# qdrant/quantization

Hardware: AMD Instinct MI355X
Metric: scored vectors/sec, 10Mx768 u8 dot (higher is better)
Workload: dtype u8; 1 GPU; 10000000 x 768 store: f32 U[0,1) -> scalar u8 (dot); per step: encode_query + score_all over the shard; quantizer=u8, rows_per_gpu=10000000, dim=768, distance=dot, exchange=scores, gather_group=1, launch=single rank, world_size_seen=1, encode_ahead=False, total_rows=10000000, queries=16

## Files before the change

### quantization_amd/csrc/u8.hip

```cpp
#include <algorithm>
#include <cmath>
#include <cstdlib>
#include <memory>
#include <vector>

#include "common.hpp"
#include "lists.hpp"
#include "multi_reduce.hpp"
#include "topk.hpp"
#include "topk_device.hpp"
#include "rescore.hpp"
#include "u8_internal.hpp"

#pragma clang fp contract(off)

using namespace qamd;

namespace {

constexpr int kBlock = 256;
constexpr int kScanBlock = 512;
constexpr uint64_t kRowPad = 1024;
constexpr uint64_t kQuantileSample = 100000;

enum Epilogue : int { EPI_POINT = 0, EPI_INTERNAL = 1 };

typedef uint32_t u32x4 __attribute__((ext_vector_type(4)));
typedef float f32x4 __attribute__((ext_vector_type(4)));

__device__ __forceinline__ uint4 ld_nt(const uint4 *p) {
    u32x4 t = __builtin_nontemporal_load(reinterpret_cast<const u32x4 *>(p));
    return make_uint4(t.x, t.y, t.z, t.w);
}
__device__ __forceinline__ float4 ld_nt(const float4 *p) {
    f32x4 t = __builtin_nontemporal_load(reinterpret_cast<const f32x4 *>(p));
    return make_float4(t.x, t.y, t.z, t.w);
}

__device__ __forceinline__ uint32_t dot16(const uint4 &a, const uint4 &b, uint32_t acc) {
    acc = __builtin_amdgcn_udot4(a.x, b.x, acc, false);
    acc = __builtin_amdgcn_udot4(a.y, b.y, acc, false);
    acc = __builtin_amdgcn_udot4(a.z, b.z, acc, false);
    acc = __builtin_amdgcn_udot4(a.w, b.w, acc, false);
    return acc;
}

__device__ __forceinline__ uint32_t sad16(const uint4 &a, const uint4 &b, uint32_t acc) {
    acc = __builtin_amdgcn_sad_u8(a.x, b.x, acc);
    acc = __builtin_amdgcn_sad_u8(a.y, b.y, acc);
    acc = __builtin_amdgcn_sad_u8(a.z, b.z, acc);
    acc = __builtin_amdgcn_sad_u8(a.w, b.w, acc);
    return acc;
}

template <int CTRL> __device__ __forceinline__ uint32_t dpp_add(uint32_t v) {
    return v + (uint32_t)__builtin_amdgcn_update_dpp(0, (int)v, CTRL, 0xF, 0xF, false);
}
template <int G> __device__ __forceinline__ uint32_t group_sum(uint32_t v) {
    static_assert(G == 1 || G == 2 || G == 4 || G == 8 || G == 16, "row group is at most one DPP row");
    if (G >= 2) v = dpp_add<0xB1>(v);
    if (G >= 4) v = dpp_add<0x4E>(v);
    if (G >= 8) v = dpp_add<0x141>(v);
    if (G >= 16) v = dpp_add<0x140>(v);
    return v;
}

__device__ __forceinline__ float epilogue_f(float multiplier, float sf, float q_off, float v_off, float diff, int mode) {
    float ms = multiplier * sf;
    if (mode == EPI_POINT) return (ms + q_off) + v_off;
    return ms + ((q_off + v_off) - diff);
}
__device__ __forceinline__ float epilogue(float multiplier, uint32_t s, float q_off, float v_off,
                                          float diff, int mode) {
    return epilogue_f(multiplier, (float)(int32_t)s, q_off, v_off, diff, mode);
}

__device__ __forceinline__ void dot16_lanes(const uint4 &v, const uint4 &q, uint32_t (&acc)[8]) {
    const uint32_t vd[4] = {v.x, v.y, v.z, v.w};
    const uint32_t qd[4] = {q.x, q.y, q.z, q.w};
#pragma unroll
    for (int j = 0; j < 4; j++) {
        acc[2 * j] = __builtin_amdgcn_udot4(vd[j], qd[j] & 0x0000FFFFu, acc[2 * j], false);
        acc[2 * j + 1] = __builtin_amdgcn_udot4(vd[j], qd[j] & 0xFFFF0000u, acc[2 * j + 1], false);
    }
}
template <int G> __device__ __forceinline__ float avx2_lane_sum(uint32_t (&acc)[8]) {
    float f[8];
#pragma unroll
    for (int k = 0; k < 8; k++) f[k] = (float)(int32_t)group_sum<G>(acc[k]);
    float a0 = f[0] + f[4], a1 = f[1] + f[5], a2 = f[2] + f[6], a3 = f[3] + f[7];
    return (a0 + a2) + (a1 + a3);
}

__device__ __forceinline__ uint32_t f32_to_u8(float v, float alpha, float offset) {
    float x = (v - offset) / alpha;
    x = (x < 0.0f) ? 0.0f : x;
    x = (x > 127.0f) ? 127.0f : x;
    return (x != x) ? 0u : (uint32_t)x;
}

__device__ __forceinline__ bool quant_decided(float y) {
    constexpr float kBand = 3.0517578125e-05f;
    const float fr = __builtin_amdgcn_fractf(y);
    return (__builtin_fabsf(fr - 0.5f) <= 0.5f - kBand) || (__builtin_fabsf(y - 64.0f) >= 64.0f + kBand);
}
__device__ __forceinline__ uint32_t quant_code(float y) {
    return (uint32_t)__builtin_amdgcn_fmed3f(y, 0.0f, 127.0f);
}
__device__ __forceinline__ uint32_t f32x4_to_u8x4_fast(const float4 &f, float alpha, float offset, float r_alpha) {
    const float y0 = (f.x - offset) * r_alpha, y1 = (f.y - offset) * r_alpha, y2 = (f.z - offset) * r_alpha,
                y3 = (f.w - offset) * r_alpha;
    if (quant_decided(y0) && quant_decided(y1) && quant_decided(y2) && quant_decided(y3))
        return quant_code(y0) | (quant_code(y1) << 8) | (quant_code(y2) << 16) | (quant_code(y3) << 24);
    return f32_to_u8(f.x, alpha, offset) | (f32_to_u8(f.y, alpha, offset) << 8) | (f32_to_u8(f.z, alpha, offset) << 16) |
           (f32_to_u8(f.w, alpha, offset) << 24);
}

template <int G, int ITERS, int UNROLL, bool IS_L1, bool EXACT, bool FILTER, bool PACKED = false>
__global__ __launch_bounds__(kScanBlock) void u8_scan_kernel(
    const uint4 *__restrict__ codes, const float *__restrict__ offsets,
    const uint4 *__restrict__ qcodes, const float *__restrict__ q_off_p, float multiplier,
    uint32_t n_rows, uint32_t row_chunks, uint32_t n_extra, float *__restrict__ out, TopkFilter filt) {
    static_assert(!(PACKED && IS_L1), "the packed image serves Dot and L2 only");
    constexpr int RW = 64 / G;
    constexpr int TILE = RW * UNROLL;
    const int lane = threadIdx.x & 63;
    const int sub = lane % G;
    const int rslot = lane / G;
    const uint64_t wave = ((uint64_t)blockIdx.x * kScanBlock + threadIdx.x) >> 6;
    const uint64_t base = wave * TILE;
    if (base >= n_rows) return;

    uint4 v[UNROLL][ITERS];
#pragma unroll
    for (int u = 0; u < UNROLL; u++) {
        const uint64_t row = base + u * RW + rslot;
        const uint4 *p = codes + row * row_chunks;
#pragma unroll
        for (int it = 0; it < ITERS; it++) {
            const uint32_t c = sub + it * G;
            if (EXACT) {
                v[u][it] = ld_nt(p + c);
            } else if (PACKED) {
                v[u][it] = ld_nt(p + (it < ITERS - 1 || c < row_chunks ? c : row_chunks - 1));
            } else {
                const uint32_t cc = c < row_chunks ? c : row_chunks - 1;
                uint4 t = ld_nt(p + cc);
                const bool in = c < row_chunks;
                v[u][it] = make_uint4(in ? t.x : 0, in ? t.y : 0, in ? t.z : 0, in ? t.w : 0);
            }
        }
    }
    uint4 q[ITERS];
#pragma unroll
    for (int it = 0; it < ITERS; it++) {
        const uint32_t c = sub + it * G;
        if (EXACT) {
            q[it] = qcodes[c];
        } else {
            const uint4 t = qcodes[c < row_chunks ? c : row_chunks - 1];
            const bool in = c < row_chunks;
            q[it] = make_uint4(in ? t.x : 0, in ? t.y : 0, in ? t.z : 0, in ? t.w : 0);
        }
    }
    uint4 qx[PACKED ? ITERS : 1];
    uint32_t qsh[PACKED ? ITERS : 1];
    if (PACKED) {
#pragma unroll
        for (int it = 0; it < ITERS; it++) {
            const uint32_t c = sub + it * G, e = c / 7;
            const bool has = c < 7 * n_extra;
            const uint4 t = qcodes[has ? row_chunks + e : 0];
            qx[it] = make_uint4(has ? t.x : 0, has ? t.y : 0, has ? t.z : 0, has ? t.w : 0);
            qsh[it] = 7 - (c - 7 * e);
        }
    }
    const float q_off = *q_off_p;
    constexpr int NGROUPS = (UNROLL + G - 1) / G;
    float v_off[NGROUPS];
#pragma unroll
    for (int g = 0; g < NGROUPS; g++)
        v_off[g] = offsets[base + (uint64_t)(g * G + sub) * RW + rslot];
    float mine = 0.0f;
    uint32_t pivot = 0;
    if (FILTER) pivot = *filt.pivot_key;
#pragma unroll
    for (int u = 0; u < UNROLL; u++) {
        uint32_t acc = 0;
#pragma unroll
        for (int it = 0; it < ITERS; it++) {
            if (PACKED) {
                const uint4 &w = v[u][it];
                const uint32_t hi = dot16(make_uint4(w.x & 0x80808080u, w.y & 0x80808080u, w.z & 0x80808080u,
                                                     w.w & 0x80808080u), qx[it], 0);
                acc = dot16(make_uint4(w.x & 0x7F7F7F7Fu, w.y & 0x7F7F7F7Fu, w.z & 0x7F7F7F7Fu, w.w & 0x7F7F7F7Fu),
                            q[it], acc) + (hi >> qsh[it]);
            } else {
                acc = IS_L1 ? sad16(v[u][it], q[it], acc) : dot16(v[u][it], q[it], acc);
            }
        }
        acc = group_sum<G>(acc);
        if (sub == (u % G)) mine = epilogue(multiplier, acc, q_off, v_off[u / G], 0.0f, EPI_POINT);
        if ((u % G) == G - 1 || u == UNROLL - 1) {
            constexpr int dummy = 0;
            (void)dummy;
            const int first = (u / G) * G;
            const uint64_t row = base + (uint64_t)(first + sub) * RW + rslot;
            if (sub <= u - first && row < n_rows) {
                if (FILTER) topk_offer(filt, pivot, mine, (uint32_t)row);
                else __builtin_nontemporal_store(mine, out + row);
            }
        }
    }
}

template <int G, int ITERS, int UNROLL, int NQ, bool IS_L1, bool EXACT, bool FILTER>
__global__ __launch_bounds__(kScanBlock) void u8_scan_multi_kernel(
    const uint4 *__restrict__ codes, const float *__restrict__ offsets, const uint8_t *__restrict__ qcodes,
    uint32_t q_pitch, const float *__restrict__ q_offs, uint32_t nq_valid ,
    float multiplier, uint32_t n_rows, uint32_t row_chunks, float *__restrict__ out ,
    uint64_t out_pitch, TopkFilterSlices slices) {
    static_assert(G >= NQ, "one lane of the row group per query");
    constexpr int RW = 64 / G;
    constexpr int TILE = RW * UNROLL;
    constexpr int TPW = NQ;
    const int lane = threadIdx.x & 63;
    const int sub = lane % G, rslot = lane / G;
    const uint64_t wave = ((uint64_t)blockIdx.x * kScanBlock + threadIdx.x) >> 6;
    if (wave * TILE * TPW >= n_rows) return;
    uint4 q[NQ][ITERS];
#pragma unroll
    for (int j = 0; j < NQ; j++) {
        const uint4 *qj = reinterpret_cast<const uint4 *>(qcodes + (size_t)((uint32_t)j < nq_valid ? j : nq_valid - 1) * q_pitch);
#pragma unroll
        for (int it = 0; it < ITERS; it++) {
            const uint32_t c = sub + it * G;
            const bool in = EXACT || c < row_chunks;
            const uint4 t = qj[in ? c : row_chunks - 1];
            q[j][it] = make_uint4(in ? t.x : 0, in ? t.y : 0, in ? t.z : 0, in ? t.w : 0);
        }
    }
    const int my_q = multi_query_of<NQ>(sub);
    const bool owner = sub < NQ && (uint32_t)my_q < nq_valid;
    const float q_off = q_offs[owner ? my_q : 0];
    for (int tile = 0; tile < TPW; tile++) {
        const uint64_t base = (wave * TPW + tile) * TILE;
        if (base >= n_rows) break;
        uint4 v[UNROLL][ITERS];
#pragma unroll
        for (int u = 0; u < UNROLL; u++) {
            const uint4 *p = codes + (base + u * RW + rslot) * row_chunks;
#pragma unroll
            for (int it = 0; it < ITERS; it++) {
                const uint32_t c = sub + it * G;
                const bool in = EXACT || c < row_chunks;
                const uint4 t = ld_nt(p + (in ? c : row_chunks - 1));
                v[u][it] = make_uint4(in ? t.x : 0, in ? t.y : 0, in ? t.z : 0, in ? t.w : 0);
            }
        }
#pragma unroll
        for (int u = 0; u < UNROLL; u++) {
            const uint64_t row = base + (uint64_t)u * RW + rslot;
            const float v_off = offsets[row];
            uint32_t acc[NQ];
#pragma unroll
            for (int j = 0; j < NQ; j++) {
                acc[j] = 0;
#pragma unroll
                for (int it = 0; it < ITERS; it++)
                    acc[j] = IS_L1 ? sad16(v[u][it], q[j][it], acc[j]) : dot16(v[u][it], q[j][it], acc[j]);
            }
            const float mine = epilogue(multiplier, multi_reduce<G, NQ>(acc, sub), q_off, v_off, 0.0f, EPI_POINT);
            if (owner && row < n_rows) {
                if (FILTER) {
                    const TopkFilter f = topk_filter_of(slices, (uint32_t)my_q);
                    topk_offer(f, *f.pivot_key, mine, (uint32_t)row);
                } else {
                    __builtin_nontemporal_store(mine, out + (uint64_t)my_q * out_pitch + row);
                }
            }
        }
    }
}

template <int G, int ITERS, bool IS_L1, bool EXACT>
__device__ __forceinline__ void u8_topk_small_body(const uint4 *__restrict__ codes, const float *__restrict__ offsets,
                                                   const uint4 (&q)[ITERS], float q_off, float multiplier, uint32_t n_rows,
                                                   uint32_t row_chunks, uint32_t rows_per_wg, const SmallTopk &p,
                                                   unsigned long long (*lds)[64]) {
    unsigned long long(*lists)[64] = lds;
    constexpr int RW = 64 / G;
    constexpr int UNROLL = 2;
    const int lane = threadIdx.x & 63, wave = threadIdx.x >> 6;
    const int sub = lane % G, rslot = lane / G;
    unsigned long long *stage = lds[kSmallTopkWaves + wave];
// ... 558 lines not shown
#pragma unroll
    for (int m = 1; m < 64; m <<= 1) {
        s1 += __shfl_xor(s1, m, 64);
        s2 += __shfl_xor(s2, m, 64);
    }
    if (lane == 0) {
        float off;
        if (distance == QAMD_DOT) {
            float s = (float)s1;
            if (s1 >= (1u << 24)) {
                s = 0.0f;
                for (uint32_t j = 0; j < actual_dim; j++)
                    s += (float)(j < qdim ? f32_to_u8(query[j], alpha, offset) : pad_code);
            }
            off = s * alpha * offset;
        } else if (distance == QAMD_L1) {
            off = 0.0f;
        } else {
            float s = (float)s2;
            if (s2 >= (1u << 24)) {
                s = 0.0f;
                for (uint32_t j = 0; j < actual_dim; j++) {
                    float c = (float)(j < qdim ? f32_to_u8(query[j], alpha, offset) : pad_code);
                    s += c * c;
                }
            }
            off = s * alpha * alpha;
        }
        offsets_out[blockIdx.x] = invert ? -off : off;
    }
}

__global__ __launch_bounds__(kBlock) void split_rows_kernel(const uint32_t *__restrict__ rows32,
                                                           uint64_t n_rows, uint32_t row_dwords,
                                                           uint32_t *__restrict__ codes32,
                                                           float *__restrict__ offsets) {
    const uint64_t total = n_rows * row_dwords;
    const uint64_t stride = (uint64_t)gridDim.x * kBlock;
    for (uint64_t t = (uint64_t)blockIdx.x * kBlock + threadIdx.x; t < total; t += stride) {
        uint64_t r = t / row_dwords;
        uint32_t k = (uint32_t)(t - r * row_dwords);
        uint32_t w = rows32[t];
        if (k == 0)
            offsets[r] = __uint_as_float(w);
        else
            codes32[r * (row_dwords - 1) + (k - 1)] = w;
    }
}

__global__ __launch_bounds__(kBlock) void join_rows_kernel(const uint32_t *__restrict__ codes32,
                                                          const float *__restrict__ offsets,
                                                          uint64_t n_rows, uint32_t row_dwords,
                                                          uint32_t *__restrict__ rows32) {
    const uint64_t total = n_rows * row_dwords;
    const uint64_t stride = (uint64_t)gridDim.x * kBlock;
    for (uint64_t t = (uint64_t)blockIdx.x * kBlock + threadIdx.x; t < total; t += stride) {
        uint64_t r = t / row_dwords;
        uint32_t k = (uint32_t)(t - r * row_dwords);
        rows32[t] = k == 0 ? __float_as_uint(offsets[r]) : codes32[r * (row_dwords - 1) + (k - 1)];
    }
}

__global__ __launch_bounds__(kBlock) void u8_pack7_kernel(const uint4 *__restrict__ codes, uint64_t n_rows,
                                                          uint32_t row_chunks, uint32_t pchunks, uint32_t n_extra,
                                                          uint4 *__restrict__ packed, uint32_t *__restrict__ bad) {
    const uint64_t total = n_rows * pchunks, stride = (uint64_t)gridDim.x * kBlock;
    uint32_t high = 0;
    for (uint64_t t = (uint64_t)blockIdx.x * kBlock + threadIdx.x; t < total; t += stride) {
        const uint64_t r = t / pchunks;
        const uint32_t j = (uint32_t)(t - r * pchunks);
        const uint4 *row = codes + r * row_chunks;
        const uint4 a = row[j];
        uint32_t w[4] = {a.x & 0x7F7F7F7Fu, a.y & 0x7F7F7F7Fu, a.z & 0x7F7F7F7Fu, a.w & 0x7F7F7F7Fu};
        high |= a.x | a.y | a.z | a.w;
        if (j < 7 * n_extra) {
            const uint4 x = row[pchunks + j / 7];
            const uint32_t b = j % 7;
            high |= x.x | x.y | x.z | x.w;
            w[0] |= ((x.x >> b) & 0x01010101u) << 7;
            w[1] |= ((x.y >> b) & 0x01010101u) << 7;
            w[2] |= ((x.z >> b) & 0x01010101u) << 7;
            w[3] |= ((x.w >> b) & 0x01010101u) << 7;
        }
        packed[t] = make_uint4(w[0], w[1], w[2], w[3]);
    }
    if (high & 0x80808080u) atomicOr(bad, 1u);
}

int grid_for(uint64_t work_items, uint64_t per_block, int blocks_per_cu) {
    uint64_t want = (work_items + per_block - 1) / per_block;
    uint64_t cap = (uint64_t)device_info().cu_count * blocks_per_cu;
    if (want < 1) want = 1;
    return (int)(want > cap ? cap : want);
}

float host_multiplier(float alpha, int distance, int invert) {
    float m = distance == QAMD_DOT ? alpha * alpha : distance == QAMD_L1 ? alpha : -2.0f * alpha * alpha;
    return invert ? -m : m;
}

uint64_t actual_dim_of(uint64_t dim) { return dim + (16 - dim % 16) % 16; }

}


namespace {

qamd_status alloc_store(qamd_u8 *h) {
    h->padded_rows = round_up(h->count, kRowPad) + kRowPad;
    h->row_chunks = (uint32_t)(h->meta.actual_dim / 16);
    QAMD_TRY(h->codes.alloc_zero_tail(h->padded_rows * h->meta.actual_dim, h->count * h->meta.actual_dim));
    QAMD_TRY(h->offsets.alloc_zero_tail(h->padded_rows * sizeof(float), h->count * sizeof(float)));
    return QAMD_OK;
}

qamd_status build_packed(qamd_u8 *h, hipStream_t s) {
    h->packed.release();
    h->packed_chunks = 0;
    const uint32_t rc = h->row_chunks, n_extra = rc / 8, pchunks = rc - n_extra;
    if (!u8_packed_allowed() || h->count == 0 || rc < 8 || rc > 128 ||
        h->meta.vector_parameters.distance_type == QAMD_L1)
        return QAMD_OK;
    const uint64_t bytes = h->padded_rows * pchunks * 16;
    size_t free_b = 0, total_b = 0;
    if (hipMemGetInfo(&free_b, &total_b) != hipSuccess || free_b < 2 * bytes) {
        (void)hipGetLastError();
        return QAMD_OK;
    }
    DevBuf img, bad;
    const std::string err = last_error();
    if (img.alloc_zero_tail(bytes, h->count * pchunks * 16) != QAMD_OK || bad.alloc(sizeof(uint32_t), true) != QAMD_OK) {
        (void)hipGetLastError();
        last_error() = err;
        return QAMD_OK;
    }
    hipLaunchKernelGGL(u8_pack7_kernel, dim3(grid_for(h->count * pchunks, kBlock, 8)), dim3(kBlock), 0, s,
                       h->codes.as<uint4>(), h->count, rc, pchunks, n_extra, img.as<uint4>(), bad.as<uint32_t>());
    QAMD_HIP(hipGetLastError());
    uint32_t high = 0;
    QAMD_HIP(hipMemcpyAsync(&high, bad.ptr, sizeof(high), hipMemcpyDeviceToHost, s));
    QAMD_HIP(hipStreamSynchronize(s));
    if (high) return QAMD_OK;
    h->packed = std::move(img);
    h->packed_chunks = pchunks;
    return QAMD_OK;
}

template <bool IS_L1> struct ScanLaunch {
    template <int G, int ITERS, int UNROLL>
    static void go(const qamd_u8 *h, bool packed, uint32_t chunks, const uint4 *qc, const float *qo, float *out,
                   const TopkFilter *filt, hipStream_t s) {
        constexpr int TILE = (64 / G) * UNROLL;
        const uint64_t waves = (h->count + TILE - 1) / TILE;
        const unsigned grid = (unsigned)((waves + kScanBlock / 64 - 1) / (kScanBlock / 64));
        const bool exact = chunks == (uint32_t)(G * ITERS);
        const uint4 *codes = packed ? h->packed.as<uint4>() : h->codes.as<uint4>();
        const uint32_t n_extra = h->row_chunks - chunks;
#define QAMD_U8_GO(EX, FI, PK)                                                                                  \
    hipLaunchKernelGGL((u8_scan_kernel<G, ITERS, UNROLL, IS_L1, EX, FI, PK>), dim3(grid),                      \
                       dim3(kScanBlock), 0, s, codes, h->offsets.as<float>(), qc, qo, h->meta.multiplier,          \
                       (uint32_t)h->count, chunks, n_extra, out, filt ? *filt : TopkFilter{})
        if constexpr (!IS_L1) {
            if (packed) {
                if (filt) {
                    if (exact) QAMD_U8_GO(true, true, true);
                    else QAMD_U8_GO(false, true, true);
                } else {
                    if (exact) QAMD_U8_GO(true, false, true);
                    else QAMD_U8_GO(false, false, true);
                }
                return;
            }
        }
        if (filt) {
            if (exact) QAMD_U8_GO(true, true, false);
            else QAMD_U8_GO(false, true, false);
        } else {
            if (exact) QAMD_U8_GO(true, false, false);
            else QAMD_U8_GO(false, false, false);
        }
#undef QAMD_U8_GO
    }
};

template <bool IS_L1>
bool launch_scan(const qamd_u8 *h, const uint4 *qc, const float *qo, float *out, const TopkFilter *filt,
                 hipStream_t s) {
    using L = ScanLaunch<IS_L1>;
    const bool packed = !IS_L1 && h->packed_chunks != 0;
    const uint32_t rc = packed ? h->packed_chunks : h->row_chunks;
    h->last_scan_packed.store(packed ? 1 : 0, std::memory_order_relaxed);
    if (rc == 1) return L::template go<1, 1, 4>(h, packed, rc, qc, qo, out, filt, s), true;
    if (rc == 2) return L::template go<2, 1, 4>(h, packed, rc, qc, qo, out, filt, s), true;
    if (rc <= 4) return L::template go<4, 1, 8>(h, packed, rc, qc, qo, out, filt, s), true;
    if (rc <= 8) return L::template go<8, 1, 8>(h, packed, rc, qc, qo, out, filt, s), true;
    switch ((rc + 15) / 16) {
        case 1: return L::template go<16, 1, 8>(h, packed, rc, qc, qo, out, filt, s), true;
        case 2: return L::template go<16, 2, 4>(h, packed, rc, qc, qo, out, filt, s), true;
        case 3: return L::template go<16, 3, 4>(h, packed, rc, qc, qo, out, filt, s), true;
        case 4: return L::template go<16, 4, 2>(h, packed, rc, qc, qo, out, filt, s), true;
        case 5: return L::template go<16, 5, 2>(h, packed, rc, qc, qo, out, filt, s), true;
        case 6: return L::template go<16, 6, 2>(h, packed, rc, qc, qo, out, filt, s), true;
        case 7: return L::template go<16, 7, 2>(h, packed, rc, qc, qo, out, filt, s), true;
        case 8: return L::template go<16, 8, 2>(h, packed, rc, qc, qo, out, filt, s), true;
        default: break;
    }
    return false;
}

template <bool IS_L1>
void launch_scan_generic(const qamd_u8 *h, const uint4 *qc, const float *qo, float *out, hipStream_t s) {
    uint64_t waves = (h->count + 3) / 4;
    unsigned grid = (unsigned)((waves + kBlock / 64 - 1) / (kBlock / 64));
    hipLaunchKernelGGL((u8_scan_generic_kernel<IS_L1>), dim3(grid), dim3(kBlock), 0, s,
                       h->codes.as<uint4>(), h->offsets.as<float>(), qc, qo, h->meta.multiplier,
                       (uint32_t)h->count, h->row_chunks, out);
}

template <bool IS_L1> struct SmallLaunch {
    template <int G, int ITERS>
    static qamd_status go(const qamd_u8 *h, const uint4 *qc, const float *qo, const FusedQuery *fq, const SmallTopkPlan &pl,
                          const SmallTopk &p, hipStream_t s) {
        const bool exact = h->row_chunks == (uint32_t)(G * ITERS);
        if constexpr (G * ITERS * 16 > (int)kFusedQueryDims + 15 * 16) {
            if (fq) return fail(QAMD_ERR_ARGUMENTS, "fused query does not fit the kernel arguments");
        } else if (fq) {
            QueryByValue qv;
            memcpy(qv.v, fq->values, (size_t)fq->qdim * 4);
            const qamd_vector_parameters &vp = h->meta.vector_parameters;
#define QAMD_U8_SMALL_FUSED(EX)                                                                                        \
    hipLaunchKernelGGL((u8_topk_small_fused_kernel<G, ITERS, IS_L1, EX>), dim3(pl.workgroups), dim3(1024), 0, s,          \
                       h->codes.as<uint4>(), h->offsets.as<float>(), qv, fq->qdim, (uint32_t)h->meta.actual_dim,         \
                       h->meta.alpha, h->meta.offset, vp.distance_type, vp.invert, fq->qbuf, h->meta.multiplier,           \
                       (uint32_t)h->count, h->row_chunks, pl.rows_per_wg, p)
            if (exact) QAMD_U8_SMALL_FUSED(true);
            else QAMD_U8_SMALL_FUSED(false);
#undef QAMD_U8_SMALL_FUSED
            QAMD_HIP(hipGetLastError());
            return QAMD_OK;
        }
#define QAMD_U8_SMALL(EX)                                                                                       \
    hipLaunchKernelGGL((u8_topk_small_kernel<G, ITERS, IS_L1, EX>), dim3(pl.workgroups), dim3(1024), 0, s,       \
                       h->codes.as<uint4>(), h->offsets.as<float>(), qc, qo, h->meta.multiplier, (uint32_t)h->count, \
                       h->row_chunks, pl.rows_per_wg, p)
        if (exact) QAMD_U8_SMALL(true);
        else QAMD_U8_SMALL(false);
#undef QAMD_U8_SMALL
        QAMD_HIP(hipGetLastError());
        return QAMD_OK;
    }
};

int small_group(uint32_t rc) { return rc == 1 ? 1 : rc == 2 ? 2 : rc <= 4 ? 4 : rc <= 8 ? 8 : rc <= 128 ? 16 : 0; }

template <bool IS_L1>
qamd_status launch_small(const qamd_u8 *h, const uint4 *qc, const float *qo, const FusedQuery *fq, const SmallTopkPlan &pl,
                         const SmallTopk &p, hipStream_t s) {
    using L = SmallLaunch<IS_L1>;
    const uint32_t rc = h->row_chunks;
    h->last_scan_packed.store(0, std::memory_order_relaxed);
    if (rc == 1) return L::template go<1, 1>(h, qc, qo, fq, pl, p, s);
    if (rc == 2) return L::template go<2, 1>(h, qc, qo, fq, pl, p, s);
    if (rc <= 4) return L::template go<4, 1>(h, qc, qo, fq, pl, p, s);
    if (rc <= 8) return L::template go<8, 1>(h, qc, qo, fq, pl, p, s);
    switch ((rc + 15) / 16) {
        case 1: return L::template go<16, 1>(h, qc, qo, fq, pl, p, s);
        case 2: return L::template go<16, 2>(h, qc, qo, fq, pl, p, s);
        case 3: return L::template go<16, 3>(h, qc, qo, fq, pl, p, s);
        case 4: return L::template go<16, 4>(h, qc, qo, fq, pl, p, s);
        case 5: return L::template go<16, 5>(h, qc, qo, fq, pl, p, s);
        case 6: return L::template go<16, 6>(h, qc, qo, fq, pl, p, s);
        case 7: return L::template go<16, 7>(h, qc, qo, fq, pl, p, s);
        case 8: return L::template go<16, 8>(h, qc, qo, fq, pl, p, s);
        default: break;
    }
    return fail(QAMD_ERR_ARGUMENTS, "no small top-k kernel for %u chunks", rc);
}

template <bool IS_L1, int G, int ITERS, int UNROLL, int NQ>
void launch_multi_shape(const qamd_u8 *h, const uint8_t *qcodes, uint64_t q_pitch, const float *q_offs, uint32_t nq_valid,
                        float *out, const TopkFilterSlices *slices, hipStream_t s) {
    constexpr int TILE = (64 / G) * UNROLL * NQ;
    const uint64_t waves = (h->count + TILE - 1) / TILE;
    const unsigned grid = (unsigned)((waves + kScanBlock / 64 - 1) / (kScanBlock / 64));
    const bool exact = h->row_chunks == (uint32_t)(G * ITERS);
    h->last_scan_packed.store(0, std::memory_order_relaxed);
#define QAMD_U8_MULTI(EX, FI)                                                                                      \
// ... 1028 lines not shown
                                uint32_t n_queries, uint32_t k, int largest, uint32_t *out_ids, float *out_scores,
                                qamd_mem out_mem, hipStream_t stream) {
    auto qc = [&](uint32_t q) { return reinterpret_cast<const uint4 *>(codes_dev + (uint64_t)q * pitch); };
    BatchScan scan;
    scan.filter_capable = fused_capable(h);
    scan.scan_scores = [&](uint32_t q, float *scores, hipStream_t st) { return scan_ptrs(h, qc(q), offsets_dev + q, scores, st); };
    scan.scan_filter = [&](uint32_t q, const TopkFilter &f, hipStream_t st) {
        return scan_ptrs(h, qc(q), offsets_dev + q, nullptr, st, &f);
    };
    scan.score_ids = [&](uint32_t q, const uint32_t *ids, uint64_t n_ids, float *out, hipStream_t st) {
        return score_ids_dev(h, qc(q), offsets_dev + q, 0.0f, EPI_POINT, ids, n_ids, out, st);
    };
    const bool is_l1 = h->meta.vector_parameters.distance_type == QAMD_L1;
    const uint32_t width = multi_width(h);
    if (width)
        scan.scan_filter_multi = [&, width, is_l1](uint32_t q, uint32_t left, const TopkFilterSlices &sl, hipStream_t st,
                                                   qamd_status &status) -> uint32_t {
            const uint32_t nq = std::min(left, width);
            if (nq < 2) return 0;
            const uint8_t *qcodes = codes_dev + (uint64_t)q * pitch;
            const bool ok = is_l1 ? launch_multi<true>(h, nq, qcodes, pitch, offsets_dev + q, nullptr, &sl, st)
                                  : launch_multi<false>(h, nq, qcodes, pitch, offsets_dev + q, nullptr, &sl, st);
            if (ok && hipGetLastError() != hipSuccess) status = fail(QAMD_ERR_DEVICE, "u8 multi-query filter launch failed");
            return ok ? nq : 0;
        };
    return fused_topk_batch(h->count, n_queries, k, largest, out_ids, out_scores, out_mem, stream, scan);
}

bool u8_host_encode_is_lazy(uint64_t qdim) { return qdim > 0 && actual_dim_of(qdim) <= kFusedQueryDims; }

qamd_status u8_score_lists(const qamd_u8 *h, const uint8_t *codes_dev, uint64_t pitch, const float *offsets_dev,
                           const ListArgs &a, hipStream_t stream) {
    return score_pairs_dev(h, nullptr, nullptr, codes_dev, (uint32_t)pitch, offsets_dev, a.offsets, a.n_lists, nullptr, 0.0f,
                           EPI_POINT, a.ids, a.n_pairs, a.out, stream);
}

uint32_t u8_multi_width(const qamd_u8 *h) { return multi_width(h); }

bool u8_lane_order(const qamd_u8 *h) { return lane_order(h); }

qamd_status u8_score_batch_scans(const qamd_u8 *h, const uint8_t *codes_dev, uint64_t pitch, const float *offsets_dev,
                                 uint32_t n_queries, float *out_dev, hipStream_t stream) {
    const bool is_l1 = h->meta.vector_parameters.distance_type == QAMD_L1;
    const uint32_t width = multi_width(h);
    uint32_t q = 0;
    while (q < n_queries) {
        const uint32_t nq = std::min(width, n_queries - q);
        const uint8_t *qcodes = codes_dev + (uint64_t)q * pitch;
        float *o = out_dev + (uint64_t)q * h->count;
        const bool ok = nq >= 2 && (is_l1 ? launch_multi<true>(h, nq, qcodes, pitch, offsets_dev + q, o, nullptr, stream)
                                          : launch_multi<false>(h, nq, qcodes, pitch, offsets_dev + q, o, nullptr, stream));
        if (ok) {
            q += nq;
        } else {
            QAMD_TRY(scan_ptrs(h, reinterpret_cast<const uint4 *>(qcodes), offsets_dev + q, o, stream));
            q += 1;
        }
    }
    QAMD_HIP(hipGetLastError());
    return QAMD_OK;
}

qamd_status u8_topk_single(const qamd_u8 *h, const uint8_t *codes_dev, const float *offset_dev, uint32_t k,
                           int largest, uint32_t *out_ids, float *out_scores, qamd_mem out_mem, hipStream_t stream) {
    return u8_topk_ptrs(h, codes_dev, offset_dev, k, largest, out_ids, out_scores, out_mem, stream, nullptr);
}

qamd_status u8_score_single(const qamd_u8 *h, const uint8_t *codes_dev, const float *offset_dev, float *out_dev,
                            hipStream_t stream) {
    return scan_ptrs(h, reinterpret_cast<const uint4 *>(codes_dev), offset_dev, out_dev, stream);
}

}

#ifdef QAMD_DEV
extern "C" __attribute__((visibility("default"))) void qamd_dev_u8_ptrs(const qamd_u8 *h, const void **codes,
                                                                        const void **offsets) {
    *codes = h->codes.ptr;
    *offsets = h->offsets.ptr;
}
extern "C" __attribute__((visibility("default"))) const void *qamd_dev_u8_query_ptr(const qamd_u8_query *q) {
    return q->buf.ptr;
}
extern "C" __attribute__((visibility("default"))) void qamd_dev_u8_packed(const qamd_u8 *h, const void **packed,
                                                                          uint32_t *chunks) {
    *packed = h->packed.ptr;
    *chunks = h->packed_chunks;
}
extern "C" __attribute__((visibility("default"))) int qamd_dev_u8_last_scan_packed(const qamd_u8 *h) {
    return h->last_scan_packed.load(std::memory_order_relaxed);
}
#endif

extern "C" qamd_status qamd_u8_topk_rescored(const qamd_u8 *h, const qamd_u8_query *q, const qamd_f32 *orig,
                                              const float *query_f32, uint64_t qdim, qamd_mem query_mem, uint32_t k,
                                              uint32_t candidates, int largest, uint32_t *out_ids, float *out_scores,
                                              qamd_mem out_mem, void *stream) {
    if (!h || !q) return qamd::fail(QAMD_ERR_ARGUMENTS, "null handle or query");
    return qamd::topk_rescored(h->device, h->meta.vector_parameters, orig, query_f32, 1, qdim, query_mem, k, candidates, largest, out_ids,
                               out_scores, out_mem, qamd::as_stream(stream), [&](uint32_t *ids_dev, float *scores_dev) {
                                   return qamd_u8_topk(h, q, candidates, largest, ids_dev, scores_dev, QAMD_MEM_DEVICE, stream);
                               });
}
```

### quantization_amd/csrc/u8_internal.hpp

```cpp
#pragma once
#include <atomic>
#include <mutex>

#include "common.hpp"
#include "lists.hpp"

struct qamd_u8 {
    int device = 0;
    qamd_u8_metadata meta{};
    uint64_t count = 0;
    uint64_t padded_rows = 0;
    uint32_t row_chunks = 0;
    int lane_mode = 0;
    qamd::DevBuf codes;
    qamd::DevBuf offsets;
    qamd::DevBuf packed;
    uint32_t packed_chunks = 0;
    mutable std::atomic<int> last_scan_packed{0};
    mutable std::mutex sample_mu;
    mutable qamd::DevBuf sample_codes, sample_offsets;
    mutable uint32_t sample_rows = 0;
};

struct qamd_u8_query {
    int device = 0;
    uint64_t actual_dim = 0;
    qamd::DevBuf buf;
    mutable qamd::ReadyEvent ready;
    mutable std::vector<float> host_f32;
    float alpha = 0.0f, offset = 0.0f;
    int distance = 0, invert = 0;
    mutable std::atomic<bool> deferred{false};
    mutable std::mutex encode_mu;
    bool pooled = false;
    mutable std::atomic<bool> async_used{false};
    ~qamd_u8_query() {
        if (pooled) qamd::query_buf_put(buf, !async_used.load(std::memory_order_relaxed) && ready.complete());
    }
};

namespace qamd {
qamd_status u8_minmax_range(const float *data, qamd_mem mem, uint64_t n_rows, uint64_t dim, hipStream_t s, float *mn,
                            float *mx);
qamd_status u8_quantile_interval(const float *data, qamd_mem mem, uint64_t count, uint64_t dim, float quantile,
                                 hipStream_t s, bool *found, float *mn, float *mx);
}

namespace qamd {
qamd_status u8_encode_queries_device(const qamd_u8 *h, const float *queries_dev, uint64_t n_queries, uint64_t qdim,
                                     uint8_t *codes_dev , uint64_t code_pitch,
                                     float *offsets_dev ,
                                     hipStream_t stream);
bool u8_host_encode_is_lazy(uint64_t qdim);
struct FusedQuery {
    const float *values = nullptr;
    uint32_t qdim = 0;
    uint8_t *qbuf = nullptr;
};
qamd_status u8_topk_ptrs(const qamd_u8 *h, const uint8_t *codes_dev, const float *offset_dev, uint32_t k, int largest,
                         uint32_t *out_ids, float *out_scores, qamd_mem out_mem, hipStream_t stream,
                         const FusedQuery *fq = nullptr);
qamd_status u8_topk_batch_scans(const qamd_u8 *h, const uint8_t *codes_dev, uint64_t pitch, const float *offsets_dev,
                                uint32_t n_queries, uint32_t k, int largest, uint32_t *out_ids, float *out_scores,
                                qamd_mem out_mem, hipStream_t stream);
uint32_t u8_multi_width(const qamd_u8 *h);
bool u8_lane_order(const qamd_u8 *h);
qamd_status u8_score_batch_scans(const qamd_u8 *h, const uint8_t *codes_dev, uint64_t pitch, const float *offsets_dev,
                                 uint32_t n_queries, float *out_dev, hipStream_t stream);
qamd_status u8_score_single(const qamd_u8 *h, const uint8_t *codes_dev, const float *offset_dev, float *out_dev,
                            hipStream_t stream);
qamd_status u8_score_lists(const qamd_u8 *h, const uint8_t *codes_dev, uint64_t pitch, const float *offsets_dev,
                           const ListArgs &a, hipStream_t stream);
qamd_status u8_topk_single(const qamd_u8 *h, const uint8_t *codes_dev, const float *offset_dev, uint32_t k,
                           int largest, uint32_t *out_ids, float *out_scores, qamd_mem out_mem, hipStream_t stream);
}
```

Baseline: 9.635 billion vectors/s.

## Store packed u8 image in 64-row blocked layout and scan with dedicated kernel

```diff
diff --git a/quantization_amd/csrc/u8.hip b/quantization_amd/csrc/u8.hip
--- a/quantization_amd/csrc/u8.hip
+++ b/quantization_amd/csrc/u8.hip
@@ -2,6 +2,7 @@
 #include <cmath>
 #include <cstdlib>
 #include <memory>
+#include <type_traits>
 #include <vector>
 
 #include "common.hpp"
@@ -116,12 +117,11 @@
            (f32_to_u8(f.w, alpha, offset) << 24);
 }
 
-template <int G, int ITERS, int UNROLL, bool IS_L1, bool EXACT, bool FILTER, bool PACKED = false>
+template <int G, int ITERS, int UNROLL, bool IS_L1, bool EXACT, bool FILTER>
 __global__ __launch_bounds__(kScanBlock) void u8_scan_kernel(
     const uint4 *__restrict__ codes, const float *__restrict__ offsets,
     const uint4 *__restrict__ qcodes, const float *__restrict__ q_off_p, float multiplier,
-    uint32_t n_rows, uint32_t row_chunks, uint32_t n_extra, float *__restrict__ out, TopkFilter filt) {
-    static_assert(!(PACKED && IS_L1), "the packed image serves Dot and L2 only");
+    uint32_t n_rows, uint32_t row_chunks, float *__restrict__ out, TopkFilter filt) {
     constexpr int RW = 64 / G;
     constexpr int TILE = RW * UNROLL;
     const int lane = threadIdx.x & 63;
@@ -141,8 +141,6 @@
             const uint32_t c = sub + it * G;
             if (EXACT) {
                 v[u][it] = ld_nt(p + c);
-            } else if (PACKED) {
-                v[u][it] = ld_nt(p + (it < ITERS - 1 || c < row_chunks ? c : row_chunks - 1));
             } else {
                 const uint32_t cc = c < row_chunks ? c : row_chunks - 1;
                 uint4 t = ld_nt(p + cc);
@@ -163,18 +161,6 @@
             q[it] = make_uint4(in ? t.x : 0, in ? t.y : 0, in ? t.z : 0, in ? t.w : 0);
         }
     }
-    uint4 qx[PACKED ? ITERS : 1];
-    uint32_t qsh[PACKED ? ITERS : 1];
-    if (PACKED) {
-#pragma unroll
-        for (int it = 0; it < ITERS; it++) {
-            const uint32_t c = sub + it * G, e = c / 7;
-            const bool has = c < 7 * n_extra;
-            const uint4 t = qcodes[has ? row_chunks + e : 0];
-            qx[it] = make_uint4(has ? t.x : 0, has ? t.y : 0, has ? t.z : 0, has ? t.w : 0);
-            qsh[it] = 7 - (c - 7 * e);
-        }
-    }
     const float q_off = *q_off_p;
     constexpr int NGROUPS = (UNROLL + G - 1) / G;
     float v_off[NGROUPS];
@@ -188,17 +174,7 @@
     for (int u = 0; u < UNROLL; u++) {
         uint32_t acc = 0;
 #pragma unroll
-        for (int it = 0; it < ITERS; it++) {
-            if (PACKED) {
-                const uint4 &w = v[u][it];
-                const uint32_t hi = dot16(make_uint4(w.x & 0x80808080u, w.y & 0x80808080u, w.z & 0x80808080u,
-                                                     w.w & 0x80808080u), qx[it], 0);
-                acc = dot16(make_uint4(w.x & 0x7F7F7F7Fu, w.y & 0x7F7F7F7Fu, w.z & 0x7F7F7F7Fu, w.w & 0x7F7F7F7Fu),
-                            q[it], acc) + (hi >> qsh[it]);
-            } else {
-                acc = IS_L1 ? sad16(v[u][it], q[it], acc) : dot16(v[u][it], q[it], acc);
-            }
-        }
+        for (int it = 0; it < ITERS; it++) acc = IS_L1 ? sad16(v[u][it], q[it], acc) : dot16(v[u][it], q[it], acc);
         acc = group_sum<G>(acc);
         if (sub == (u % G)) mine = epilogue(multiplier, acc, q_off, v_off[u / G], 0.0f, EPI_POINT);
         if ((u % G) == G - 1 || u == UNROLL - 1) {
@@ -211,6 +187,83 @@
                 else __builtin_nontemporal_store(mine, out + row);
             }
         }
+    }
+}
+
+constexpr uint32_t kPackBlockRows = 64;
+constexpr uint32_t kPackBlockChunk = kPackBlockRows;
+
+__device__ __forceinline__ uint4 and16(const uint4 &v, uint32_t m) { return make_uint4(v.x & m, v.y & m, v.z & m, v.w & m); }
+
+template <bool FILTER>
+__global__ __launch_bounds__(kScanBlock) __attribute__((amdgpu_waves_per_eu(8, 8))) void u8_scan_blocked_kernel(
+    const uint4 *__restrict__ image, const float *__restrict__ offsets, const uint4 *__restrict__ qcodes,
+    const float *__restrict__ q_off_p, float multiplier, uint32_t n_rows, uint32_t pchunks, uint32_t n_extra,
+    uint32_t split, float *__restrict__ out, TopkFilter filt) {
+    __shared__ uint32_t partial[kScanBlock];
+    const uint32_t lane = threadIdx.x & 63;
+    const uint32_t wave = __builtin_amdgcn_readfirstlane(threadIdx.x >> 6);
+    const uint32_t part = wave & (split - 1);
+    const uint64_t block = (uint64_t)blockIdx.x * ((kScanBlock / 64) / split) + wave / split;
+    const uint64_t row = block * kPackBlockRows + lane;
+    const bool live = block * kPackBlockRows < n_rows;
+    const uint32_t n_rest = pchunks - 7 * n_extra, n_groups = n_extra + (n_rest ? 1 : 0);
+    const uint32_t g_begin = live ? n_groups * part / split : 0, g_end = live ? n_groups * (part + 1) / split : 0;
+    const uint4 *blk = image + block * pchunks * kPackBlockChunk;
+    const uint32_t lane16 = lane * 16;
+    auto chunk_ptr = [&](uint32_t c) {
+        return reinterpret_cast<const uint4 *>(reinterpret_cast<const char *>(blk + (uint64_t)c * kPackBlockChunk) + lane16);
+    };
+    const uint32_t gf_end = g_end < n_extra ? g_end : n_extra;
+    const bool has_rest = g_end > n_extra;
+
+    uint4 v[7];
+    uint32_t acc = 0;
+    auto eat = [&](uint32_t g, auto refill) {
+        const uint4 *q = qcodes + 7 * g;
+        const uint4 qx = qcodes[pchunks + g];
+#pragma unroll
+        for (int i = 0; i < 7; i++) {
+            const uint4 w = v[i];
+            acc = dot16(and16(w, 0x7F7F7F7Fu), q[i], acc) + (dot16(and16(w, 0x80808080u), qx, 0) >> (7 - i));
+            if (decltype(refill)::value) {
+                __builtin_amdgcn_sched_barrier(0);
+                v[i] = ld_nt(chunk_ptr(7 * (g + 1) + i));
+                __builtin_amdgcn_sched_barrier(0);
+            }
+        }
+    };
+    if (g_begin < gf_end) {
+#pragma unroll
+        for (int i = 0; i < 7; i++) v[i] = ld_nt(chunk_ptr(7 * g_begin + i));
+    }
+    const float v_off = offsets[row];
+    const float q_off = *q_off_p;
+    uint32_t pivot = 0;
+    if (FILTER) pivot = *filt.pivot_key;
+    if (g_begin < gf_end) {
+        for (uint32_t g = g_begin; g + 1 < gf_end; g++) eat(g, std::true_type{});
+        eat(gf_end - 1, std::false_type{});
+    }
+    if (has_rest) {
+        const uint4 *q = qcodes + 7 * n_extra;
+#pragma unroll
+        for (int i = 0; i < 7; i++)
+            if ((uint32_t)i < n_rest) v[i] = ld_nt(chunk_ptr(7 * n_extra + i));
+#pragma unroll
+        for (int i = 0; i < 7; i++)
+            if ((uint32_t)i < n_rest) acc = dot16(and16(v[i], 0x7F7F7F7Fu), q[i], acc);
+    }
+    if (split > 1) {
+        partial[threadIdx.x] = acc;
+        __syncthreads();
+        if (part == 0)
+            for (uint32_t p = 1; p < split; p++) acc += partial[threadIdx.x + 64 * p];
+    }
+    if (part == 0 && row < n_rows) {
+        const float score = epilogue(multiplier, acc, q_off, v_off, 0.0f, EPI_POINT);
+        if (FILTER) topk_offer(filt, pivot, score, (uint32_t)row);
+        else __builtin_nontemporal_store(score, out + row);
     }
 }
 
@@ -935,7 +988,7 @@
             w[2] |= ((x.z >> b) & 0x01010101u) << 7;
             w[3] |= ((x.w >> b) & 0x01010101u) << 7;
         }
-        packed[t] = make_uint4(w[0], w[1], w[2], w[3]);
+        packed[((r / kPackBlockRows) * pchunks + j) * kPackBlockRows + r % kPackBlockRows] = make_uint4(w[0], w[1], w[2], w[3]);
     }
     if (high & 0x80808080u) atomicOr(bad, 1u);
 }
@@ -969,6 +1022,7 @@
 
 qamd_status build_packed(qamd_u8 *h, hipStream_t s) {
     h->packed.release();
+    h->packed_rows.release();
     h->packed_chunks = 0;
     const uint32_t rc = h->row_chunks, n_extra = rc / 8, pchunks = rc - n_extra;
     if (!u8_packed_allowed() || h->count == 0 || rc < 8 || rc > 128 ||
@@ -982,7 +1036,7 @@
     }
     DevBuf img, bad;
     const std::string err = last_error();
-    if (img.alloc_zero_tail(bytes, h->count * pchunks * 16) != QAMD_OK || bad.alloc(sizeof(uint32_t), true) != QAMD_OK) {
+    if (img.alloc_zero_tail(bytes, h->count / kPackBlockRows * kPackBlockRows * pchunks * 16) != QAMD_OK || bad.alloc(sizeof(uint32_t), true) != QAMD_OK) {
         (void)hipGetLastError();
         last_error() = err;
         return QAMD_OK;
@@ -1001,61 +1055,70 @@
 
 template <bool IS_L1> struct ScanLaunch {
     template <int G, int ITERS, int UNROLL>
-    static void go(const qamd_u8 *h, bool packed, uint32_t chunks, const uint4 *qc, const float *qo, float *out,
-                   const TopkFilter *filt, hipStream_t s) {
+    static void go(const qamd_u8 *h, const uint4 *qc, const float *qo, float *out, const TopkFilter *filt, hipStream_t s) {
         constexpr int TILE = (64 / G) * UNROLL;
         const uint64_t waves = (h->count + TILE - 1) / TILE;
         const unsigned grid = (unsigned)((waves + kScanBlock / 64 - 1) / (kScanBlock / 64));
-        const bool exact = chunks == (uint32_t)(G * ITERS);
-        const uint4 *codes = packed ? h->packed.as<uint4>() : h->codes.as<uint4>();
-        const uint32_t n_extra = h->row_chunks - chunks;
-#define QAMD_U8_GO(EX, FI, PK)                                                                                  \
-    hipLaunchKernelGGL((u8_scan_kernel<G, ITERS, UNROLL, IS_L1, EX, FI, PK>), dim3(grid),                      \
-                       dim3(kScanBlock), 0, s, codes, h->offsets.as<float>(), qc, qo, h->meta.multiplier,          \
-                       (uint32_t)h->count, chunks, n_extra, out, filt ? *filt : TopkFilter{})
-        if constexpr (!IS_L1) {
-            if (packed) {
-                if (filt) {
-                    if (exact) QAMD_U8_GO(true, true, true);
-                    else QAMD_U8_GO(false, true, true);
-                } else {
-                    if (exact) QAMD_U8_GO(true, false, true);
-                    else QAMD_U8_GO(false, false, true);
-                }
-                return;
-            }
-        }
+        const bool exact = h->row_chunks == (uint32_t)(G * ITERS);
+#define QAMD_U8_GO(EX, FI)                                                                                     \
+    hipLaunchKernelGGL((u8_scan_kernel<G, ITERS, UNROLL, IS_L1, EX, FI>), dim3(grid), dim3(kScanBlock), 0, s,    \
+                       h->codes.as<uint4>(), h->offsets.as<float>(), qc, qo, h->meta.multiplier, (uint32_t)h->count, \
+                       h->row_chunks, out, filt ? *filt : TopkFilter{})
         if (filt) {
-            if (exact) QAMD_U8_GO(true, true, false);
-            else QAMD_U8_GO(false, true, false);
+            if (exact) QAMD_U8_GO(true, true);
+            else QAMD_U8_GO(false, true);
         } else {
-            if (exact) QAMD_U8_GO(true, false, false);
-            else QAMD_U8_GO(false, false, false);
+            if (exact) QAMD_U8_GO(true, false);
+            else QAMD_U8_GO(false, false);
         }
 #undef QAMD_U8_GO
     }
 };
+
+uint32_t blocked_split(uint64_t count) {
+    const uint64_t blocks = (count + kPackBlockRows - 1) / kPackBlockRows;
+    const uint64_t want = (uint64_t)device_info().cu_count * 16;
+    uint32_t split = 1;
+    while (split < 8 && blocks * split < want) split *= 2;
+    return split;
+}
+
+void launch_scan_blocked(const qamd_u8 *h, const uint4 *qc, const float *qo, float *out, const TopkFilter *filt,
+                         hipStream_t s) {
+    const uint32_t split = blocked_split(h->count), blocks_per_wg = (kScanBlock / 64) / split;
+    const uint64_t blocks = (h->count + kPackBlockRows - 1) / kPackBlockRows;
+    const unsigned grid = (unsigned)((blocks + blocks_per_wg - 1) / blocks_per_wg);
+    h->last_scan_split.store((int)split, std::memory_order_relaxed);
+#define QAMD_U8_BLOCKED(FI)                                                                                          \
+    hipLaunchKernelGGL((u8_scan_blocked_kernel<FI>), dim3(grid), dim3(kScanBlock), 0, s, h->packed.as<uint4>(),       \
+                       h->offsets.as<float>(), qc, qo, h->meta.multiplier, (uint32_t)h->count, h->packed_chunks,      \
+                       h->row_chunks - h->packed_chunks, split, out, filt ? *filt : TopkFilter{})
+    if (filt) QAMD_U8_BLOCKED(true);
+    else QAMD_U8_BLOCKED(false);
+#undef QAMD_U8_BLOCKED
+}
 
 template <bool IS_L1>
 bool launch_scan(const qamd_u8 *h, const uint4 *qc, const float *qo, float *out, const TopkFilter *filt,
                  hipStream_t s) {
     using L = ScanLaunch<IS_L1>;
     const bool packed = !IS_L1 && h->packed_chunks != 0;
-    const uint32_t rc = packed ? h->packed_chunks : h->row_chunks;
     h->last_scan_packed.store(packed ? 1 : 0, std::memory_order_relaxed);
-    if (rc == 1) return L::template go<1, 1, 4>(h, packed, rc, qc, qo, out, filt, s), true;
-    if (rc == 2) return L::template go<2, 1, 4>(h, packed, rc, qc, qo, out, filt, s), true;
-    if (rc <= 4) return L::template go<4, 1, 8>(h, packed, rc, qc, qo, out, filt, s), true;
-    if (rc <= 8) return L::template go<8, 1, 8>(h, packed, rc, qc, qo, out, filt, s), true;
+    if (packed) return launch_scan_blocked(h, qc, qo, out, filt, s), true;
+    const uint32_t rc = h->row_chunks;
+    if (rc == 1) return L::template go<1, 1, 4>(h, qc, qo, out, filt, s), true;
+    if (rc == 2) return L::template go<2, 1, 4>(h, qc, qo, out, filt, s), true;
+    if (rc <= 4) return L::template go<4, 1, 8>(h, qc, qo, out, filt, s), true;
+    if (rc <= 8) return L::template go<8, 1, 8>(h, qc, qo, out, filt, s), true;
     switch ((rc + 15) / 16) {
-        case 1: return L::template go<16, 1, 8>(h, packed, rc, qc, qo, out, filt, s), true;
-        case 2: return L::template go<16, 2, 4>(h, packed, rc, qc, qo, out, filt, s), true;
-        case 3: return L::template go<16, 3, 4>(h, packed, rc, qc, qo, out, filt, s), true;
-        case 4: return L::template go<16, 4, 2>(h, packed, rc, qc, qo, out, filt, s), true;
-        case 5: return L::template go<16, 5, 2>(h, packed, rc, qc, qo, out, filt, s), true;
-        case 6: return L::template go<16, 6, 2>(h, packed, rc, qc, qo, out, filt, s), true;
-        case 7: return L::template go<16, 7, 2>(h, packed, rc, qc, qo, out, filt, s), true;
-        case 8: return L::template go<16, 8, 2>(h, packed, rc, qc, qo, out, filt, s), true;
+        case 1: return L::template go<16, 1, 8>(h, qc, qo, out, filt, s), true;
+        case 2: return L::template go<16, 2, 4>(h, qc, qo, out, filt, s), true;
+        case 3: return L::template go<16, 3, 4>(h, qc, qo, out, filt, s), true;
+        case 4: return L::template go<16, 4, 2>(h, qc, qo, out, filt, s), true;
+        case 5: return L::template go<16, 5, 2>(h, qc, qo, out, filt, s), true;
+        case 6: return L::template go<16, 6, 2>(h, qc, qo, out, filt, s), true;
+        case 7: return L::template go<16, 7, 2>(h, qc, qo, out, filt, s), true;
+        case 8: return L::template go<16, 8, 2>(h, qc, qo, out, filt, s), true;
         default: break;
     }
     return false;
@@ -2250,10 +2313,43 @@
 extern "C" __attribute__((visibility("default"))) const void *qamd_dev_u8_query_ptr(const qamd_u8_query *q) {
     return q->buf.ptr;
 }
+namespace {
+__global__ __launch_bounds__(kBlock) void u8_unblock_kernel(const uint4 *__restrict__ image, uint64_t n_rows,
+                                                            uint32_t pchunks, uint4 *__restrict__ rows) {
+    const uint64_t total = n_rows * pchunks, stride = (uint64_t)gridDim.x * kBlock;
+    for (uint64_t t = (uint64_t)blockIdx.x * kBlock + threadIdx.x; t < total; t += stride) {
+        const uint64_t r = t / pchunks;
+        const uint32_t j = (uint32_t)(t - r * pchunks);
+        rows[t] = image[((r / kPackBlockRows) * pchunks + j) * kPackBlockRows + r % kPackBlockRows];
+    }
+}
+}
 extern "C" __attribute__((visibility("default"))) void qamd_dev_u8_packed(const qamd_u8 *h, const void **packed,
                                                                           uint32_t *chunks) {
+    *packed = nullptr;
+    *chunks = 0;
+    if (!h->packed_chunks) return;
+    if (!h->packed_rows.ptr) {
+        const uint64_t n = h->count * h->packed_chunks;
+        if (h->packed_rows.alloc(n * 16, false) != QAMD_OK) return;
+        hipLaunchKernelGGL(u8_unblock_kernel, dim3(grid_for(n, kBlock, 8)), dim3(kBlock), 0, nullptr, h->packed.as<uint4>(),
+                           h->count, h->packed_chunks, h->packed_rows.as<uint4>());
+        if (hipStreamSynchronize(nullptr) != hipSuccess) {
+            h->packed_rows.release();
+            return;
+        }
+    }
+    *packed = h->packed_rows.ptr;
+    *chunks = h->packed_chunks;
+}
+extern "C" __attribute__((visibility("default"))) void qamd_dev_u8_packed_blocked(const qamd_u8 *h, const void **packed,
+                                                                                  uint32_t *chunks, uint32_t *block_rows) {
     *packed = h->packed.ptr;
     *chunks = h->packed_chunks;
+    *block_rows = kPackBlockRows;
+}
+extern "C" __attribute__((visibility("default"))) int qamd_dev_u8_last_scan_split(const qamd_u8 *h) {
+    return h->last_scan_split.load(std::memory_order_relaxed);
 }
 extern "C" __attribute__((visibility("default"))) int qamd_dev_u8_last_scan_packed(const qamd_u8 *h) {
     return h->last_scan_packed.load(std::memory_order_relaxed);
diff --git a/quantization_amd/csrc/u8_internal.hpp b/quantization_amd/csrc/u8_internal.hpp
--- a/quantization_amd/csrc/u8_internal.hpp
+++ b/quantization_amd/csrc/u8_internal.hpp
@@ -17,6 +17,8 @@
     qamd::DevBuf packed;
     uint32_t packed_chunks = 0;
     mutable std::atomic<int> last_scan_packed{0};
+    mutable std::atomic<int> last_scan_split{0};
+    mutable qamd::DevBuf packed_rows;
     mutable std::mutex sample_mu;
     mutable qamd::DevBuf sample_codes, sample_offsets;
     mutable uint32_t sample_rows = 0;
```

New measurement: 9.962 billion vectors/s (median of 6 runs). +3.4%, better.
